# TrevorS/voxtral-mini-realtime-rs

Measured on AMD Instinct MI355X. Metric: decode_tok_per_s, higher is better.
Workload: dtype f32

## Files before the change

voxtral-mini-realtime-rs_amd/csrc/vox_engine.hip:

```cpp
#include "vox_kernels.h"

#include <hip/hip_fp16.h>

#include <cstdio>
#include <cstdlib>

namespace vox {
namespace {

#include "vox_engine_common.h"

__global__ __launch_bounds__(64) void eng_pack_lm_kernel(Q4W w, unsigned char* __restrict__ stream, size_t op_off, int vocab) {
    const int q = blockIdx.x, b = blockIdx.y, lane = threadIdx.x;
    const int row = lm_rows_per_cu(vocab) * b + q;
    unsigned char* dst = stream + (size_t)NCU * (op_off + (size_t)(q / NCONS) * PK_A) + (size_t)b * PK_A + (size_t)(q % NCONS) * PASS_A;
    const size_t src = (size_t)row * w.nb + lane;
    reinterpret_cast<uint4*>(dst)[lane] = w.qs[src];
    reinterpret_cast<uint16_t*>(dst + PA_S0)[lane] = w.sc[src];
    const size_t sh = (size_t)row * w.nb + 64 + (lane >> 1);
    const uint4 qh = w.qs[sh];
    reinterpret_cast<uint2*>(dst + PA_Q1)[lane] = (lane & 1) ? make_uint2(qh.z, qh.w) : make_uint2(qh.x, qh.y);
    if ((lane & 1) == 0) reinterpret_cast<uint16_t*>(dst + PA_S1)[lane >> 1] = w.sc[sh];
}
__global__ __launch_bounds__(64) void eng_pack_kernel(Q4W w, int op, unsigned char* __restrict__ stream, size_t op_off) {
// ... 125 lines not shown
    const EngLayerTab* tab = reinterpret_cast<const EngLayerTab*>(lds + L_TAB);
    const unsigned tag_base = (*p.serial + 1u) * 64u;
    const bool PROBE_SMALL = (p.flags & 4) != 0;
    const int own_r = min(lane0, OWN - 1);
    const unsigned own_k = (unsigned)(OWN * b + own_r);
    const float* gwt = reinterpret_cast<const float*>(lds + L_GW);
    {
        const float g0 = ld_gf(make_srd(p.n_layers > 0 ? tab[0].attn_norm : p.final_norm, ED * 4u), own_k) * (p.n_layers > 0 ? 1.0f : 512.0f);
        const float hraw = (p.flags & ENGF_ARGMAX_IN) ? comm_next_input(p, lane0, own_k) : ld_gf(make_srd(p.h_in, ED * 4u), own_k);
        comm_publish_rows(p, lane0, hraw, g0, p.H0, p.SS0, tag_base, c->h_own);
    }
#pragma unroll 1
    for (int st = 0; st <= 2 * p.n_layers; st++) {
        int lane = lane0; asm volatile("" : "+v"(lane));
        const int l = st >> 1; const bool odd = st & 1, last = st == 2 * p.n_layers, T = l == p.tl_layer;
        const unsigned tag = tag_base + (unsigned)l + 1u;
        if (odd) comm_probe_x(p, c, lane, p.H1, tag, tl, T);
        else comm_probe_x(p, c, lane, p.H0, tag - 1u, tl, false);
        lds_st(&c->gathering, 1u);
        lds_st(&c->ag_flag, (unsigned)st + 1u);
        if (T) tl(odd ? 11 : 8);
        if (p.flags & (1 | 64)) wait_ge(&c->ag_done, NCONS * ((unsigned)st + 1u), c, p.err, ERR_STAGE);
        lds_st(&c->gathering, 0u);
        if (last) break;
        if (!odd) {
            wait_ge(&c->gw_flag, (unsigned)NCONS, c, p.err, ERR_STAGE);
            const bool xloc_nt = (p.flags & 128) != 0 && (p.flags & 4096) != 0 && lds_ld(&c->xcd_ok) != 0;
            {
                wait_ge(&c->pub_cnt, NCONS * (4u * (unsigned)l + 1u), c, p.err, ERR_STAGE);
                lds_st(&c->gathering, 1u);
                float v[6];
                sweep<6>(p.G, (EQD + 2 * EKD) * 8u, tag, [&](int u) { const int i = lane + 64 * u, seg = i >> 7, e = i & 127; return seg == 0 ? 128 * h + e : (seg == 1 ? EQD : EQD + EKD) + 128 * g + e; },
                         [&]() { return lane < 32 ? EQD + 128 * g + 4 * lane : EQD + EKD + 128 * g + 4 * (lane - 32); }, PROBE_SMALL, v, c, p.err, xloc_nt);
                lds_st(&c->gathering, 0u);
#pragma unroll
                for (int u = 0; u < 6; u++) qkvn[lane + 64 * u] = v[u];
                ENG_CFENCE(); lds_st(&c->qkv_flag, (unsigned)l + 1u);
            }
            if (T) tl(9);
            {
                wait_ge(&c->pub_cnt, NCONS * (4u * (unsigned)l + 2u), c, p.err, ERR_STAGE);
                lds_st(&c->gathering, 1u);
                float v[6];
                sweep<6>(p.PW, NPW * ED * 8u, tag, [&](int u) { const int i = lane + 64 * u, hh = i / OWN, r = i - hh * OWN; return hh * ED + OWN * b + r; }, [&]() { return (lane & 31) * ED + OWN * b; }, PROBE_SMALL, v, c, p.err);
#pragma unroll
                for (int u = 0; u < 6; u++) tmp[lane + 64 * u] = v[u];
                lds_st(&c->gathering, 0u);
                ENG_CFENCE();
                float a = 0.f;
                const int r = min(lane, OWN - 1);
#pragma unroll 4
                for (int hh = 0; hh < NPW; hh++) a += tmp[hh * OWN + r];
                wait_ge(&c->gw_flag, (unsigned)NCONS, c, p.err, ERR_STAGE);
                if (!((p.flags & 16384) && blockIdx.x == 7 && l == 1))
                    comm_publish_rows(p, lane, c->h_own[r] + a, gwt[(l * 2 + 1) * 16 + r], p.H1, p.SS1, tag, c->h1_own);
            }
            if (T) tl(10);
        } else {
            const bool xloc_nt = (p.flags & 128) != 0 && (p.flags & 4096) != 0 && lds_ld(&c->xcd_ok) != 0;
            {
                wait_ge(&c->pub_cnt, NCONS * (4u * (unsigned)l + 3u), c, p.err, ERR_STAGE);
                lds_st(&c->gathering, 1u);
                float v[18];
                sweep<18>(p.A, EF * 8u, tag, [&](int u) { return 1152 * g + lane + 64 * u; }, [&]() { return 1152 * g + 36 * (lane & 31) + 35; }, PROBE_SMALL, v, c, p.err, xloc_nt);
#pragma unroll
                for (int u = 0; u < 18; u++) xa[lane + 64 * u] = v[u];
                ENG_CFENCE(); lds_st(&c->xa_flag, (unsigned)l + 1u);
                lds_st(&c->gathering, 0u);
            }
            if (T) tl(12);
            {
                wait_ge(&c->pub_cnt, NCONS * (4u * (unsigned)l + 4u), c, p.err, ERR_STAGE);
                lds_st(&c->gathering, 1u);
                float v[2];
                sweep<2>(p.P2, NP2 * ED * 8u, tag, [&](int u) { const int i = min(lane + 64 * u, NP2 * OWN - 1), pp = i / OWN, r = i - pp * OWN; return pp * ED + OWN * b + r; }, [&]() { return min(lane, NP2 - 1) * ED + OWN * b; }, PROBE_SMALL, v, c, p.err);
#pragma unroll
                for (int u = 0; u < 2; u++) if (lane + 64 * u < NP2 * OWN) tmp[lane + 64 * u] = v[u];
                lds_st(&c->gathering, 0u);
                ENG_CFENCE();
                float a = 0.f;
                const int r = min(lane, OWN - 1);
#pragma unroll
                for (int pp = 0; pp < NP2; pp++) a += tmp[pp * OWN + r];
                comm_publish_rows(p, lane, c->h1_own[r] + a, gwt[((l + 1) * 2) * 16 + r], p.H0, p.SS0, tag, c->h_own);
            }
            if (T) tl(13);
        }
    }
}

__device__ __forceinline__ f2 cvt2(unsigned w, bool hi) { return hi ? __builtin_amdgcn_cvt_pk_f32_fp8((int)w, true) : __builtin_amdgcn_cvt_pk_f32_fp8((int)w, false); }
__device__ __forceinline__ float block_dot(const uint4 q, const f2* __restrict__ x, float init) {
    f2 a0 = {init, 0.f}, a1 = {0.f, 0.f};
    const unsigned w[4] = {q.x, q.y, q.z, q.w};
#pragma unroll
    for (int d = 0; d < 4; d++) {
        const unsigned lo = w[d] & 0x0F0F0F0Fu, hi = (w[d] >> 4) & 0x0F0F0F0Fu;
        a0 = __builtin_elementwise_fma(cvt2(lo, false), x[2 * d], a0);
        a1 = __builtin_elementwise_fma(cvt2(lo, true), x[2 * d + 1], a1);
        a0 = __builtin_elementwise_fma(cvt2(hi, false), x[8 + 2 * d], a0);
        a1 = __builtin_elementwise_fma(cvt2(hi, true), x[8 + 2 * d + 1], a1);
    }
    return (a0.x + a0.y) + (a1.x + a1.y);
}

__device__ __forceinline__ float half_dot(const uint2 q, const f2* __restrict__ x, float init) {
    f2 a0 = {init, 0.f}, a1 = {0.f, 0.f};
    const unsigned w[2] = {q.x, q.y};
#pragma unroll
    for (int d = 0; d < 2; d++) {
        const unsigned lo = w[d] & 0x0F0F0F0Fu, hi = (w[d] >> 4) & 0x0F0F0F0Fu;
        a0 = __builtin_elementwise_fma(cvt2(lo, false), x[4 * d], a0);
        a1 = __builtin_elementwise_fma(cvt2(lo, true), x[4 * d + 1], a1);
        a0 = __builtin_elementwise_fma(cvt2(hi, false), x[4 * d + 2], a0);
        a1 = __builtin_elementwise_fma(cvt2(hi, true), x[4 * d + 3], a1);
    }
    return (a0.x + a0.y) + (a1.x + a1.y);
}

struct XA {
    f2 x[16], xh[8]; float m8, m8h;
    __device__ __forceinline__ void load_chunk(const float* xs, int chunk) {
        asm volatile("" : "+v"(chunk));
        const float4* x4 = reinterpret_cast<const float4*>(xs);
        float s = 0.f;
#pragma unroll
        for (int jj = 0; jj < 8; jj++) {
            const float4 v = x4[sw_piece(chunk, jj)];
            x[2 * jj] = f2{v.x, v.y}; x[2 * jj + 1] = f2{v.z, v.w};
            s += (v.x + v.y) + (v.z + v.w);
        }
        m8 = s * (-1.0f / 64.0f);
    }
    __device__ __forceinline__ void load(const float* xs, int chunk, int chunk_h, int hb) {
        load_chunk(xs, chunk);
        asm volatile("" : "+v"(chunk_h));
        const float4* x4 = reinterpret_cast<const float4*>(xs);
        float s = 0.f;
#pragma unroll
        for (int d = 0; d < 2; d++)
#pragma unroll
            for (int hh = 0; hh < 2; hh++) {
                const float4 v = x4[sw_piece(chunk_h, 4 * hh + 2 * hb + d)];
                xh[4 * d + 2 * hh] = f2{v.x, v.y}; xh[4 * d + 2 * hh + 1] = f2{v.z, v.w};
                s += (v.x + v.y) + (v.z + v.w);
            }
        m8h = s * (-1.0f / 64.0f);
    }
};
struct PassA { uint4 q0; uint2 q1; float s0, s1; };

typedef int i4v __attribute__((ext_vector_type(4)));
struct StepCtx { i4v A; float m8sx, sxinv; };
__device__ __forceinline__ StepCtx load_ctx(const unsigned char* planes, const float2* binfo, int blk0, int lane) {
    const int n = lane & 15, g = lane >> 4;
    StepCtx cx; cx.A = i4v{0, 0, 0, 0};
    if (n < 8 && (g >> 1) == (n >> 2)) cx.A = *reinterpret_cast<const i4v*>(planes + (((blk0 + (n >> 2)) * 4 + (n & 3)) * 2 + (g & 1)) * 16);
    const float2 bi = binfo[blk0 + (g & 1)];
    cx.m8sx = bi.x; cx.sxinv = bi.y;
    return cx;
}
struct RecR { i4v B; float sc; };
__device__ __forceinline__ RecR rec_read(const unsigned char* rec, bool half, int lane) {
    const int n = lane & 15, g = lane >> 4;
    uint2 q = make_uint2(0u, 0u);
    if (!half) q = reinterpret_cast<const uint2*>(rec)[lane];
    else if (n < 8) q = reinterpret_cast<const uint2*>(rec)[g * 8 + n];
    const unsigned short sb = reinterpret_cast<const unsigned short*>(rec + (half ? REC_H_SC : REC_SC))[(half ? 8 : 16) * (g & 1) + (half ? (n & 7) : n)];
    RecR r;
    r.B[0] = (int)(q.x & 0x0F0F0F0Fu); r.B[1] = (int)(q.y & 0x0F0F0F0Fu); r.B[2] = (int)((q.x >> 4) & 0x0F0F0F0Fu); r.B[3] = (int)((q.y >> 4) & 0x0F0F0F0Fu);
    r.sc = __half2float(__ushort_as_half(sb));
    asm volatile("" : "+v"(r.B[0]), "+v"(r.B[1]), "+v"(r.B[2]), "+v"(r.B[3]), "+v"(r.sc));
    return r;
}
__device__ __forceinline__ float mstep(const RecR& r, const StepCtx& cx, float acc) {
    const i4v D = __builtin_amdgcn_mfma_i32_16x16x64_i8(cx.A, r.B, i4v{0, 0, 0, 0}, 0, 0, 0);
    const int lo = (int)((unsigned)D[0] + ((unsigned)D[1] << 7)), hi = (int)((unsigned)D[2] + ((unsigned)D[3] << 7));
    float t = fmaf((float)hi, 16384.0f, (float)lo);
    t += cx.m8sx;
    return fmaf(t, r.sc * cx.sxinv, acc);
}
__device__ __forceinline__ float mstep(const unsigned char* rec, bool half, int lane, const StepCtx& cx, float acc) { return mstep(rec_read(rec, half, lane), cx, acc); }
__device__ __forceinline__ float g01_sum(float v, int lane) { return v + __shfl(v, (lane + 16) & 63); }
__device__ __forceinline__ void to_digits(const float (&v)[4], int lane, unsigned char* plane_blk, float2* binfo_blk) {
    float mx = fmaxf(fmaxf(fabsf(v[0]), fabsf(v[1])), fmaxf(fabsf(v[2]), fabsf(v[3])));
    mx = fmaxf(mx, dppf<0xB1>(mx)); mx = fmaxf(mx, dppf<0x4E>(mx)); mx = fmaxf(mx, dppf<0x141>(mx));
    int e = __builtin_amdgcn_frexp_expf(mx);
    e = max(e, -100);
    const float f = ldexpf(1.0f, 26 - e);
    int xi[4];
#pragma unroll
    for (int i = 0; i < 4; i++) xi[i] = (int)rintf(v[i] * f);
    int s = (xi[0] + xi[1]) + (xi[2] + xi[3]);
    s += dppi<0xB1>(s); s += dppi<0x4E>(s); s += dppi<0x141>(s);
    if ((lane & 7) == 0) *binfo_blk = make_float2(-8.0f * (float)s, ldexpf(1.0f, e - 26));
    const int e0 = 4 * (lane & 7), h = (e0 >> 3) & 1, off = (e0 & 4) + 8 * (e0 >> 4);
#pragma unroll
    for (int cdig = 0; cdig < 4; cdig++) {
        unsigned d = 0;
#pragma unroll
        for (int i = 0; i < 4; i++) { const int dv = cdig < 3 ? (xi[i] >> (7 * cdig)) & 127 : xi[i] >> 21; d |= (unsigned)(dv & 0xFF) << (8 * i); }
        *reinterpret_cast<unsigned*>(plane_blk + (cdig * 2 + h) * 16 + off) = d;
    }
}

struct Cons {
    const EngParams& p; EngCtl* c; unsigned char* lds; int cw, lane; unsigned P; unsigned cbar_n;
    __device__ __forceinline__ Cons(const EngParams& p_, EngCtl* c_, unsigned char* lds_, int cw_, int lane_) : p(p_), c(c_), lds(lds_), cw(cw_), lane(lane_), P(0), cbar_n(0) {}
    __device__ __forceinline__ void cbarrier() {
        cbar_n += NCONS;
        ENG_CFENCE();
        if (lane == 0) __hip_atomic_fetch_add(&c->cbar, 1u, RLX, WG);
        wait_ge(&c->cbar, cbar_n, c, p.err, ERR_CBAR);
    }
    __device__ __forceinline__ void published(const Tl& tl, int evt) {
        ENG_CFENCE();
        if (lane == 0) { const unsigned old = __hip_atomic_fetch_add(&c->pub_cnt, 1u, RLX, WG); if (evt >= 0 && tl.buf && old % NCONS == NCONS - 1) tl.buf[evt] = wall_clock64(); }
    }
    __device__ __forceinline__ const unsigned char* slot_wait(unsigned pk, int share_bytes, int& slot) {
        slot = (int)(pk % NSLOT); const unsigned k = pk / NSLOT;
        wait_ge(&c->ring_ready[slot], k + 1u, c, p.err, ERR_RING);
        return lds + L_RING + slot * SLOT_BYTES + cw * share_bytes;
    }
    __device__ __forceinline__ void slot_release(int slot) {
        ENG_CFENCE();
        if (lane == 0) __hip_atomic_fetch_add(&c->ring_done[slot], 1u, RLX, WG);
    }
    __device__ __forceinline__ void fetch(unsigned pk, PassA& P_) {
        int slot; const unsigned char* base = slot_wait(pk, PASS_A, slot);
        P_.q0 = reinterpret_cast<const uint4*>(base)[lane];
        P_.q1 = reinterpret_cast<const uint2*>(base + PA_Q1)[lane];
        P_.s0 = __half2float(__ushort_as_half(reinterpret_cast<const unsigned short*>(base + PA_S0)[lane]));
        P_.s1 = __half2float(__ushort_as_half(reinterpret_cast<const unsigned short*>(base + PA_S1)[lane >> 1]));
        slot_release(slot);
    }
    static __device__ __forceinline__ float dot(const PassA& P_, const XA& xr) { return fmaf(P_.s1, half_dot(P_.q1, xr.xh, xr.m8h), P_.s0 * block_dot(P_.q0, xr.x, xr.m8)); }

    template <bool DIGITS>
    __device__ __forceinline__ float all_gather(const u64* src, const u64* ssq, unsigned tag, unsigned stage, unsigned char* xs, float* ssl, float2* binfo, const Tl& tl, bool T) {
        wait_ge(&c->ag_flag, stage + 1u, c, p.err, ERR_STAGE);
        const srd_t sd = make_srd(src, ED * 8u), qd = make_srd(ssq, NCU * 8u);
        int ln = lane; asm volatile("" : "+v"(ln));
        if (DIGITS) {
            const unsigned q = 64u * (unsigned)cw + (unsigned)ln;
            u32x4 ra, rb; u64 rq = 0, t0 = 0;
            for (;;) {
                ra = __builtin_bit_cast(u32x4, __builtin_amdgcn_raw_buffer_load_b128(sd, (int)(q * 32u), 0, 16));
                rb = __builtin_bit_cast(u32x4, __builtin_amdgcn_raw_buffer_load_b128(sd, (int)(q * 32u + 16u), 0, 16));
                if (cw < 4) rq = ld_gran(qd, 64u * (unsigned)cw + (unsigned)ln);
                bool ok = ra.y == tag && ra.w == tag && rb.y == tag && rb.w == tag;
                if (cw < 4) ok &= (unsigned)(rq >> 32) == tag;
                if (__all(ok)) break;
                if (sweep_bail(t0, tag, c, p.err)) break;
            }
            if (T) tl(22);
            if (ln == 0) __hip_atomic_fetch_add(&c->ag_done, 1u, RLX, WG);
            const float v[4] = {__uint_as_float(ra.x), __uint_as_float(ra.z), __uint_as_float(rb.x), __uint_as_float(rb.z)};
            to_digits(v, ln, xs + (q >> 3) * 128u, binfo + (q >> 3));
            if (cw < 4) ssl[64 * cw + ln] = __uint_as_float((unsigned)rq);
            return 0.f;
        }
        const unsigned q = 64u * (((unsigned)cw + blockIdx.x) % NCONS) + (unsigned)ln;
        u32x4 ra, rb; u64 rq = 0, t0 = 0;
        for (;;) {
            ra = __builtin_bit_cast(u32x4, __builtin_amdgcn_raw_buffer_load_b128(sd, (int)(q * 32u), 0, 16));
            rb = __builtin_bit_cast(u32x4, __builtin_amdgcn_raw_buffer_load_b128(sd, (int)(q * 32u + 16u), 0, 16));
            if (cw < 4) rq = ld_gran(qd, 64u * (unsigned)cw + (unsigned)ln);
            bool ok = ra.y == tag && ra.w == tag && rb.y == tag && rb.w == tag;
            if (cw < 4) ok &= (unsigned)(rq >> 32) == tag;
            if (__all(ok)) break;
            if (sweep_bail(t0, tag, c, p.err)) break;
        }
        if (ln == 0) __hip_atomic_fetch_add(&c->ag_done, 1u, RLX, WG);
        const float v[4] = {__uint_as_float(ra.x), __uint_as_float(ra.z), __uint_as_float(rb.x), __uint_as_float(rb.z)};
#pragma unroll
        for (int i = 0; i < 4; i++) reinterpret_cast<float*>(xs)[sw_dword((int)(4u * q) + i)] = v[i];
        if (cw < 4) ssl[64 * cw + ln] = __uint_as_float((unsigned)rq);
        cbarrier();
        return rstd_staged(ssl);
    }
    __device__ __forceinline__ float rstd_staged(const float* ssl) {
        const float ss = wave_sum_e((ssl[lane] + ssl[lane + 64]) + (ssl[lane + 128] + ssl[lane + 192]));
        return 1.0f / sqrtf(ss / (float)ED + p.eps);
    }
};

__device__ __forceinline__ void eng_consumer(const EngParams& p, EngCtl* c, unsigned char* lds, int cw, const int lane0, const Tl& tl) {
    Cons cs(p, c, lds, cw, lane0);
    const int b = blockIdx.x, g = b & 7, j = b >> 3, h = 4 * g + (j >> 3), s = j & 7;
    unsigned char* xs = lds + L_XS; float* ssl = reinterpret_cast<float*>(lds + L_SSQ);
    float2* binfo = reinterpret_cast<float2*>(lds + L_BLK);
    const float* xa = reinterpret_cast<const float*>(lds + L_XA);
    float* part = reinterpret_cast<float*>(lds + L_PART);
    float* part2 = reinterpret_cast<float*>(lds + L_XA + 1152 * 4);
    const float* qkvn = reinterpret_cast<const float*>(lds + L_QKVN);
    float* sc = reinterpret_cast<float*>(lds + L_SC); float2* po = reinterpret_cast<float2*>(lds + L_PO); float* pl = reinterpret_cast<float*>(lds + L_PL);
    const unsigned tag_base = (*p.serial + 1u) * 64u;
    const int pos = *p.pos_ptr + p.pos_off + ((p.flags & ENGF_ARGMAX_IN) ? 1 : 0);
    const int j_lo = p.window >= 0 ? max(0, pos - p.window) : 0, n_old = pos - j_lo, last_old = max(n_old - 1, 0);
    const int half = EHD / 2;
    if (cw == 0 && lane0 < 24) {
        float rc = 1.0f, rs = 0.0f;
        if (lane0 < 20) { const int pr = lane0 < 16 ? 8 * s + (lane0 >> 1) : 2 * j + ((lane0 - 16) >> 1); rc = p.rope_cos[(size_t)pos * half + pr]; rs = p.rope_sin[(size_t)pos * half + pr]; }
        c->rope_c[lane0] = rc; c->rope_s[lane0] = rs;
    }
    const float scale = 1.0f / sqrtf((float)EHD);
    const int n_items = 3 * p.n_layers, npass_lm = lm_passes(p.vocab), row0_lm = lm_rows_per_cu(p.vocab) * b;
    {
        const EngLayerTab* tab = reinterpret_cast<const EngLayerTab*>(lds + L_TAB);
        float* gwt = reinterpret_cast<float*>(lds + L_GW);
        const bool xchg = cw == NCONS - 1 && (p.flags & 128) != 0;
        const unsigned my = c->xcc_id;
        if (xchg && lane0 == 0) publish(p.XC + b, tag_base, __uint_as_float(my));
        const int l = cw + NCONS * (lane0 >> 4), r = lane0 & 15, lc = min(l, max(p.n_layers - 1, 0));
        const bool lok = r < OWN && l <= p.n_layers && (lane0 >> 4) < 3, lay = l < p.n_layers;
        const unsigned k = (unsigned)(OWN * b + min(r, OWN - 1));
        const gcf_p pa = as_g(lay ? tab[lc].attn_norm : p.final_norm);
        float wa = 0.f, wf = 0.f, wd = 0.f;
        if (lok) { wa = pa[k]; if (p.n_layers > 0) { wf = as_g(tab[lc].ffn_norm)[k]; wd = as_g(tab[lc].ada_mul)[k]; } }
        if (lok) {
            gwt[(l * 2) * 16 + r] = lay ? wa : wa * 512.0f;
            if (lay) gwt[(l * 2 + 1) * 16 + r] = wf * wd;
        }
        if (cw == NCONS - 1) {
            unsigned ok = 0;
            if (xchg) {
                float v[1];
                const bool got = sweep<1>(p.XC, NCU * 8u, tag_base, [&](int) { return 8 * (lane0 & 31) + g; }, [&]() { return 0; }, false, v, c, p.err);
                ok = got && __all(__float_as_uint(v[0]) == my) ? 1u : 0u;
                if (!ok && lane0 == 0) __hip_atomic_store(p.err + 1, 9u | ((unsigned)b << 8) | (my << 16), RLX, AG);
            }
            lds_st(&c->xcd_ok, ok);
        }
        ENG_CFENCE();
        if (lane0 == 0) __hip_atomic_fetch_add(&c->gw_flag, 1u, RLX, WG);
    }
    float best = -INFINITY; int best_i = 0x7fffffff;
    bool xloc = false;

#pragma unroll 1
    for (int it = 0; it <= n_items; it++) {
        int lane = lane0; asm volatile("" : "+v"(lane));
        const int l = it / 3, op = it == n_items ? (int)EOP_LM : (it - 3 * l == 0 ? (int)EOP_QKV : it - 3 * l == 1 ? (int)EOP_W13 : (int)EOP_W2);
        const bool T = l == p.tl_layer && cw == 0 && op != EOP_LM;
        const int tlev = l == p.tl_layer ? 1 : 0;
        const unsigned tag = tag_base + (unsigned)l + 1u;
        const EngLayerTab* L = reinterpret_cast<const EngLayerTab*>(lds + L_TAB) + (op == EOP_LM ? 0 : l);
        if (op == EOP_QKV) {
            const gf_p kc = as_g(L->kc) + (size_t)g * p.max_seq * EHD, vc = as_g(L->vc) + (size_t)g * p.max_seq * EHD;
            const int t12 = cw * 64 + lane;
            const int part_ = t12 & 7, ks = t12 >> 3;
            RecR rq[8];
            {
                int s0, s1, s2;
                const unsigned char* b0 = cs.slot_wait(cs.P, 2 * REC, s0);
                rq[0] = rec_read(b0, false, lane); rq[1] = rec_read(b0 + REC, false, lane);
                cs.slot_release(s0);
                const unsigned char* b1 = cs.slot_wait(cs.P + 1, 2 * REC, s1);
                rq[2] = rec_read(b1, false, lane); rq[3] = rec_read(b1 + REC, false, lane);
                cs.slot_release(s1);
                const unsigned char* b2 = cs.slot_wait(cs.P + 2, 4 * REC_H, s2);
#pragma unroll
                for (int i = 0; i < 4; i++) rq[4 + i] = rec_read(b2 + i * REC_H, true, lane);
                cs.slot_release(s2);
                cs.P += QKV_PK;
            }
            cs.all_gather<true>(p.H0, p.SS0, tag - 1u, 2u * (unsigned)l, xs, ssl, binfo, tl, false);
            if (T) tl(0);
            constexpr int NKP = 2;
            float4 kpre[NKP][4];
            auto kload = [&](int u) {
                const unsigned ko = (unsigned)(j_lo + min(ks + 96 * u, last_old)) * EHD + part_ * 16;
#pragma unroll
                for (int e = 0; e < 4; e++) kpre[u][e] = make_float4(0.f, 0.f, 0.f, 0.f);
                if (ks + 96 * u < n_old) {
#pragma unroll
                    for (int e = 0; e < 4; e++) kpre[u][e] = ldg4(kc + (ko + 4 * e));
                }
            };
            kload(0);
            {
                float a0 = 0.f, a1 = 0.f;
#pragma unroll
                for (int i = 0; i < 4; i++) {
                    const StepCtx cx = load_ctx(xs, binfo, 2 * (4 * cw + i), lane);
                    a0 = mstep(rq[i], cx, a0); a1 = mstep(rq[4 + i], cx, a1);
                }
                a0 = g01_sum(a0, lane); a1 = g01_sum(a1, lane);
                if (lane < 16) part[lane * NCONS + cw] = a0;
                if (lane < 8) part[(16 + lane) * NCONS + cw] = a1;
            }
            cs.cbarrier();
            if (it == 0) { wait_ge(&c->gw_flag, (unsigned)NCONS, c, p.err, ERR_STAGE); xloc = (p.flags & 128) != 0 && lds_ld(&c->xcd_ok) != 0; }
            if (cw == 0) {
                const int r = min(lane, 23);
                float a = 0.f;
#pragma unroll
                for (int w = 0; w < NCONS; w++) a += part[r * NCONS + w];
                a *= cs.rstd_staged(ssl);
                const float rc = c->rope_c[r], rs = c->rope_s[r];
                const float o = dppf<0xB1>(a);
                const float y = (lane & 1) ? fmaf(o, rs, a * rc) : fmaf(-o, rs, a * rc);
                if (lane < 24) {
                    const int n = lane < 16 ? 128 * h + 16 * s + lane : lane < 20 ? EQD + 128 * g + 4 * j + (lane - 16) : EQD + EKD + 128 * g + 4 * j + (lane - 20);
                    publish_b(p.G, (EQD + 2 * EKD) * 8u, (unsigned)n, tag, y, xloc);
                    if (lane >= 16) (lane < 20 ? kc : vc)[(size_t)pos * EHD + (n & 127)] = y;
                }
            }
            cs.published(tl, tlev ? 28 : -1);
            if (T) tl(1);
            kload(1);
            float2 vpre[16];
#pragma unroll
            for (int u = 0; u < 16; u++) {
                vpre[u] = make_float2(0.f, 0.f);
                if (cw + 12 * u < n_old) {
                    const fv2 v = *(const __attribute__((address_space(1))) fv2*)(vc + ((unsigned)(j_lo + cw + 12 * u) * EHD + lane * 2));
                    vpre[u] = make_float2(v.x, v.y);
                }
            }
            wait_ge(&c->qkv_flag, (unsigned)l + 1u, c, p.err, ERR_STAGE);
            if (T) tl(2);
            {
                float qv[16];
#pragma unroll
                for (int e = 0; e < 4; e++) { const float4 v = *reinterpret_cast<const float4*>(qkvn + part_ * 16 + 4 * e); qv[4 * e] = v.x; qv[4 * e + 1] = v.y; qv[4 * e + 2] = v.z; qv[4 * e + 3] = v.w; }
                auto dot16 = [&](const float4 (&kk)[4]) {
                    float sacc = 0.f;
#pragma unroll
                    for (int e = 0; e < 4; e++) { sacc = fmaf(qv[4 * e], kk[e].x, sacc); sacc = fmaf(qv[4 * e + 1], kk[e].y, sacc); sacc = fmaf(qv[4 * e + 2], kk[e].z, sacc); sacc = fmaf(qv[4 * e + 3], kk[e].w, sacc); }
                    return group8_sum_e(sacc);
                };
#pragma unroll
                for (int u = 0; u < NKP; u++) {
                    const float sv = dot16(kpre[u]);
                    const int i = ks + 96 * u;
                    if (part_ == 0 && i < n_old) sc[i] = sv * scale;
                }
                for (int i0 = 96 * NKP; i0 < n_old; i0 += 96 * NKP) {
#pragma unroll
                    for (int u = 0; u < NKP; u++) {
                        const int i = i0 + ks + 96 * u;
                        const unsigned ko = (unsigned)(j_lo + min(i, last_old)) * EHD + part_ * 16;
#pragma unroll
                        for (int e = 0; e < 4; e++) kpre[u][e] = make_float4(0.f, 0.f, 0.f, 0.f);
                        if (i < n_old) {
#pragma unroll
                            for (int e = 0; e < 4; e++) kpre[u][e] = ldg4(kc + (ko + 4 * e));
                        }
                    }
#pragma unroll
                    for (int u = 0; u < NKP; u++) {
                        const float sv = dot16(kpre[u]);
                        const int i = i0 + ks + 96 * u;
                        if (part_ == 0 && i < n_old) sc[i] = sv * scale;
                    }
                }
                if (cw == 0) {
                    float4 kk[4];
#pragma unroll
                    for (int e = 0; e < 4; e++) kk[e] = *reinterpret_cast<const float4*>(qkvn + 128 + part_ * 16 + 4 * e);
                    const float sv = dot16(kk);
                    if (t12 == 0) sc[n_old] = sv * scale;
                }
            }
            if (T) tl(26);
            cs.cbarrier();
            if (T) tl(27);
            {
                const int n = n_old + 1;
                float mx = -INFINITY;
                for (int i = lane; i < n; i += 64) mx = fmaxf(mx, sc[i]);
                mx = wave_max_e(mx);
                float2 o = make_float2(0.f, 0.f); float lsum = 0.f;
                const int iu = cw + 12 * (lane & 15);
                const float pv = iu < n_old ? expf(sc[iu] - mx) : 0.f;
#pragma unroll
                for (int u = 0; u < 16; u++) {
                    const float pr_ = rlf(pv, u); const float2 vv = vpre[u];
                    o.x = fmaf(pr_, vv.x, o.x); o.y = fmaf(pr_, vv.y, o.y); lsum += pr_;
                }
                for (int b0 = 192; b0 < n_old; b0 += 192) {
#pragma unroll
                    for (int u = 0; u < 16; u++) {
                        vpre[u] = make_float2(0.f, 0.f);
                        if (b0 + cw + 12 * u < n_old) {
                            const fv2 v = *(const __attribute__((address_space(1))) fv2*)(vc + ((unsigned)(j_lo + b0 + cw + 12 * u) * EHD + lane * 2));
                            vpre[u] = make_float2(v.x, v.y);
                        }
                    }
                    const int ib = b0 + cw + 12 * (lane & 15);
                    const float pb = ib < n_old ? expf(sc[ib] - mx) : 0.f;
#pragma unroll
                    for (int u = 0; u < 16; u++) {
                        const float pr_ = rlf(pb, u); const float2 vv = vpre[u];
                        o.x = fmaf(pr_, vv.x, o.x); o.y = fmaf(pr_, vv.y, o.y); lsum += pr_;
                    }
                }
                if (cw == 0) {
                    const float pr_ = expf(sc[n_old] - mx); const float2 vv = *reinterpret_cast<const float2*>(qkvn + 256 + lane * 2);
                    o.x = fmaf(pr_, vv.x, o.x); o.y = fmaf(pr_, vv.y, o.y); lsum += pr_;
                }
                po[cw * 64 + lane] = o;
                if (lane == 0) pl[cw] = lsum;
            }
            if (T) tl(23);
            cs.cbarrier();
            if (T) tl(25);
            if (lane < 32) {
                const float4* po4 = reinterpret_cast<const float4*>(po);
                float4 so = make_float4(0.f, 0.f, 0.f, 0.f); float sl = 0.f;
#pragma unroll
                for (int q = 0; q < 12; q++) { const float4 a = po4[q * 32 + lane]; so.x += a.x; so.y += a.y; so.z += a.z; so.w += a.w; sl += pl[q]; }
                const float inv = 1.0f / sl;
                const float v[4] = {so.x * inv, so.y * inv, so.z * inv, so.w * inv};
                to_digits(v, lane, xs + (8 * cw + (lane >> 3)) * 128, binfo + 8 * cw + (lane >> 3));
            }
            if (T) tl(3);
            {
                StepCtx cx[2];
#pragma unroll
                for (int i = 0; i < 2; i++) cx[i] = load_ctx(xs, binfo, 8 * cw + 2 * i, lane);
#pragma unroll
                for (int i = 0; i < WO_PK; i++) {
                    int sl_; const unsigned char* bb = cs.slot_wait(cs.P + i, 2 * REC, sl_);
                    float a = mstep(bb, false, lane, cx[0], 0.f); a = mstep(bb + REC, false, lane, cx[1], a);
                    cs.slot_release(sl_);
                    a = g01_sum(a, lane);
                    if (lane < 16) publish_b(p.PW, NPW * ED * 8u, (unsigned)(h * ED + 384 * s + 16 * (2 * cw + i) + lane), tag, a, false);
                }
                cs.P += WO_PK;
                cs.published(tl, tlev ? 29 : -1);
            }
            if (T) tl(4);
            continue;
        }
        if (op == EOP_W13) {
            constexpr int NPRE = 3;
            RecR rw[4 * NPRE];
#pragma unroll
            for (int ti = 0; ti < NPRE; ti++) {
                int s0, s1;
                const unsigned char* b0 = cs.slot_wait(cs.P + 2 * ti, 2 * REC, s0);
                rw[4 * ti] = rec_read(b0, false, lane); rw[4 * ti + 1] = rec_read(b0 + REC, false, lane);
                cs.slot_release(s0);
                const unsigned char* b1 = cs.slot_wait(cs.P + 2 * ti + 1, 2 * REC, s1);
                rw[4 * ti + 2] = rec_read(b1, false, lane); rw[4 * ti + 3] = rec_read(b1 + REC, false, lane);
                cs.slot_release(s1);
            }
            cs.all_gather<true>(p.H1, p.SS1, tag, 2u * (unsigned)l + 1u, xs, ssl, binfo, tl, T);
            if (T) tl(5);
            StepCtx cx[4];
#pragma unroll
            for (int i = 0; i < 4; i++) cx[i] = load_ctx(xs, binfo, 2 * (4 * cw + i), lane);
            if (T) tl(24);
#pragma unroll
            for (int ti = 0; ti < NPRE; ti++) {
                float a = 0.f;
#pragma unroll
                for (int i = 0; i < 4; i++) a = mstep(rw[4 * ti + i], cx[i], a);
                a = g01_sum(a, lane);
                if (lane < 16) part[(16 * ti + lane) * NCONS + cw] = a;
            }
#pragma unroll 1
            for (int ti = NPRE; ti < 4; ti++) {
                int s0, s1;
                const unsigned char* b0 = cs.slot_wait(cs.P + 2 * ti, 2 * REC, s0);
                const unsigned char* b1 = cs.slot_wait(cs.P + 2 * ti + 1, 2 * REC, s1);
                float a = mstep(b0, false, lane, cx[0], 0.f); a = mstep(b0 + REC, false, lane, cx[1], a);
                a = mstep(b1, false, lane, cx[2], a); a = mstep(b1 + REC, false, lane, cx[3], a);
                cs.slot_release(s0); cs.slot_release(s1);
                a = g01_sum(a, lane);
                if (lane < 16) part[(16 * ti + lane) * NCONS + cw] = a;
            }
            {
                int s2; const unsigned char* b2 = cs.slot_wait(cs.P + 8, 4 * REC_H, s2);
                float a = 0.f;
#pragma unroll
                for (int i = 0; i < 4; i++) a = mstep(b2 + i * REC_H, true, lane, cx[i], a);
                cs.slot_release(s2);
                a = g01_sum(a, lane);
                if (lane < 8) part[(64 + lane) * NCONS + cw] = a;
            }
            cs.P += W13_PK;
            cs.cbarrier();
            if (cw < 2) {
                const int r = min(64 * cw + lane, 71);
                float a = 0.f;
#pragma unroll
                for (int w = 0; w < NCONS; w++) a += part[r * NCONS + w];
                a *= cs.rstd_staged(ssl);
                const float up = dppf<0xB1>(a);
                if ((lane & 1) == 0 && 64 * cw + lane < 72) publish_b(p.A, EF * 8u, (unsigned)(1152 * g + 36 * j + (r >> 1)), tag, silu_e(a) * up, xloc);
            }
            cs.published(tl, tlev ? 30 : -1);
            if (T) tl(6);
            continue;
        }
        if (op == EOP_W2) {
            RecR r2[9];
#pragma unroll
            for (int i = 0; i < W2_PK; i++) {
                int sl_; const unsigned char* bb = cs.slot_wait(cs.P + i, 3 * REC, sl_);
#pragma unroll
                for (int k = 0; k < 3; k++) r2[3 * i + k] = rec_read(bb + k * REC, false, lane);
                cs.slot_release(sl_);
            }
            wait_ge(&c->xa_flag, (unsigned)l + 1u, c, p.err, ERR_STAGE);
            if (T) tl(7);
            const int ksl = cw % 6, tg = cw / 6;
            if (lane < 48) {
                const float4 v4 = *reinterpret_cast<const float4*>(xa + 32 * (6 * ksl + (lane >> 3)) + 4 * (lane & 7));
                const float v[4] = {v4.x, v4.y, v4.z, v4.w};
                to_digits(v, lane, xs + (8 * cw + (lane >> 3)) * 128, binfo + 8 * cw + (lane >> 3));
            }
            StepCtx cx[3];
#pragma unroll
            for (int i = 0; i < 3; i++) cx[i] = load_ctx(xs, binfo, 8 * cw + 2 * i, lane);
#pragma unroll
            for (int i = 0; i < W2_PK; i++) {
                float a = mstep(r2[3 * i], cx[0], 0.f); a = mstep(r2[3 * i + 1], cx[1], a); a = mstep(r2[3 * i + 2], cx[2], a);
                a = g01_sum(a, lane);
                if (lane < 16) part2[(16 * (3 * tg + i) + lane) * 6 + ksl] = a;
            }
            cs.P += W2_PK;
            cs.cbarrier();
            if (cw < 2) {
                const int r = min(64 * cw + lane, 95);
                float a = 0.f;
#pragma unroll
                for (int w = 0; w < 6; w++) a += part2[r * 6 + w];
                if (64 * cw + lane < 96) publish_b(p.P2, NP2 * ED * 8u, (unsigned)(g * ED + 96 * j + r), tag, a, false);
            }
            cs.published(tl, tlev ? 31 : -1);
            if (T) tl(14);
            continue;
        }
        const float rstd = cs.all_gather<false>(p.H0, p.SS0, tag_base + (unsigned)p.n_layers, 2u * (unsigned)p.n_layers, xs, ssl, binfo, tl, false);
        XA xr; xr.load(reinterpret_cast<const float*>(xs), lane, 64 + (lane >> 1), lane & 1);
        const int n_pass = lm_packets(p.vocab);
        PassA Qa, Qb;
        cs.fetch(cs.P, Qa);
#pragma unroll 1
        for (int t = 0; t < n_pass; t++) {
            const int q = cw + NCONS * t;
            if (t + 1 < n_pass) cs.fetch(cs.P + t + 1, Qb);
            if (q < npass_lm) {
                const float r = wave_sum_e(Cons::dot(Qa, xr)) * rstd;
                const int n = row0_lm + q;
                if (p.logits_out && lane == 0) p.logits_out[n] = r;
                if (r > best || (r == best && n < best_i)) { best = r; best_i = n; }
            }
            Qa = Qb;
        }
        cs.P += (unsigned)n_pass;
    }
    if (lane0 == 0) { c->best_val[cw] = best; c->best_idx[cw] = best_i; }
    cs.cbarrier();
    if (cw == 0 && lane0 == 0) {
        float bv = c->best_val[0]; int bi = c->best_idx[0];
        for (int w = 1; w < NCONS; w++) { const float v = c->best_val[w]; const int ii = c->best_idx[w]; if (v > bv || (v == bv && ii < bi)) { bv = v; bi = ii; } }
        p.part_val[b] = bv; p.part_idx[b] = bi;
    }
    if (cw == 0) tl(15);
}

__global__ __launch_bounds__(NTHR, 1) void decode_engine_kernel(const EngParams p) {
    extern __shared__ __attribute__((aligned(16))) unsigned char lds[];
    EngCtl* c = reinterpret_cast<EngCtl*>(lds + L_CTL);
    const int tid = threadIdx.x, lane = tid & 63, wave = __builtin_amdgcn_readfirstlane(tid >> 6);
    if (tid < (int)(sizeof(EngCtl) / 4)) reinterpret_cast<unsigned*>(c)[tid] = 0u;
    for (int i = tid; i < p.n_layers * (int)(sizeof(EngLayerTab) / 8); i += NTHR) reinterpret_cast<u64*>(lds + L_TAB)[i] = reinterpret_cast<const u64*>(p.layers)[i];
    if (tid == 0) c->xcc_id = __builtin_amdgcn_s_getreg((20) | (0 << 6) | ((4 - 1) << 11));
    __syncthreads();
    Tl tl; tl.on = p.tl != nullptr && lane == 0; tl.buf = p.tl ? p.tl + (size_t)blockIdx.x * 32 : nullptr;
    if (wave == 0) {
        tl(19);
        eng_loader(p, c, (unsigned)(uintptr_t)(lds + L_RING), lane, tl);
    } else if (wave == 1) {
        eng_comm(p, c, lds, lane, tl);
        if (blockIdx.x == 0 && lane == 0) {
            const unsigned sv = *p.serial; asm volatile("" ::: "memory"); *p.serial = sv + 1u;
            if (p.flags & ENGF_ARGMAX_IN) { const int pv_ = *p.pos_rw; asm volatile("" ::: "memory"); *p.pos_rw = pv_ + 1; }
        }
    } else {
        eng_consumer(p, c, lds, wave - 2, lane, tl);
    }
}

__global__ __launch_bounds__(256) void eng_hidden_kernel(const u64* __restrict__ H, const u64* __restrict__ SS, float eps, float* __restrict__ out) {
    __shared__ float red[256];
    const int t = threadIdx.x;
    red[t] = __uint_as_float((unsigned)SS[t]);
    __syncthreads();
    for (int s = 128; s > 0; s >>= 1) { if (t < s) red[t] += red[t + s]; __syncthreads(); }
    const float rstd = 1.0f / sqrtf(red[0] / (float)ED + eps);
    const int k = blockIdx.x * 256 + t;
    out[k] = __uint_as_float((unsigned)H[k]) * (1.0f / 512.0f) * rstd;
}

}

hipError_t launch_eng_hidden(const EngParams& p, float* out, hipStream_t s) {
    const bool even = ((2 * p.n_layers) & 1) == 0;
    eng_hidden_kernel<<<dim3(ED / 256), dim3(256), 0, s>>>(even ? p.H0 : p.H1, even ? p.SS0 : p.SS1, p.eps, out);
    return hipGetLastError();
}

bool eng_geometry_ok(int D, int n_heads, int n_kv, int hd, int ffn, int vocab, int max_seq) {
    return D == ED && n_heads == ENH && n_kv == ENKV && hd == EHD && ffn == EF && vocab > 0 && vocab % NCU == 0 && max_seq > 0 && max_seq <= SC_MAX;
}
size_t eng_stream_bytes(int n_layers, int vocab) { return cu_stream_bytes(n_layers, vocab) * NCU; }
int eng_lds_bytes() { return L_TOTAL; }

static constexpr size_t ST_H0 = 0, ST_H1 = ST_H0 + (size_t)ED * 8, ST_G = ST_H1 + (size_t)ED * 8, ST_PW = ST_G + (size_t)(EQD + 2 * EKD) * 8,
                        ST_A = ST_PW + (size_t)NPW * ED * 8, ST_P2 = ST_A + (size_t)EF * 8, ST_SS0 = ST_P2 + (size_t)NP2 * ED * 8, ST_SS1 = ST_SS0 + (size_t)NCU * 8, ST_XC = ST_SS1 + (size_t)NCU * 8, ST_SERIAL = ST_XC + (size_t)NCU * 8, ST_ERR = ST_SERIAL + 256, ST_TOTAL = ST_ERR + 256;
size_t eng_state_bytes() { return ST_TOTAL; }
void eng_state_carve(unsigned char* st, EngParams* p) {
    p->H0 = reinterpret_cast<unsigned long long*>(st + ST_H0); p->H1 = reinterpret_cast<unsigned long long*>(st + ST_H1);
    p->XC = reinterpret_cast<unsigned long long*>(st + ST_XC);
    p->SS0 = reinterpret_cast<unsigned long long*>(st + ST_SS0); p->SS1 = reinterpret_cast<unsigned long long*>(st + ST_SS1);
    p->G = reinterpret_cast<unsigned long long*>(st + ST_G); p->PW = reinterpret_cast<unsigned long long*>(st + ST_PW);
    p->A = reinterpret_cast<unsigned long long*>(st + ST_A); p->P2 = reinterpret_cast<unsigned long long*>(st + ST_P2);
    p->serial = reinterpret_cast<unsigned*>(st + ST_SERIAL); p->err = reinterpret_cast<unsigned*>(st + ST_ERR);
}

hipError_t launch_eng_pack(const Q4W& w, int op, int layer, int n_layers, unsigned char* stream, int vocab, hipStream_t s) {
    if (w.fmt != WFMT_Q4_0 || !w.qs || !w.sc) return hipErrorInvalidValue;
    int off_bytes, N, K;
    switch (op) {
    case EOP_QKV: off_bytes = OFF_QKV; N = EQD + 2 * EKD; K = ED; break;
    case EOP_WO: off_bytes = OFF_WO; N = ED; K = EQD; break;
    case EOP_W13: off_bytes = OFF_W13; N = 2 * EF; K = ED; break;
    case EOP_W2: off_bytes = OFF_W2; N = ED; K = EF; break;
    case EOP_LM: off_bytes = 0; N = vocab; K = ED; break;
    case EOP_WOB: off_bytes = 0; N = ED; K = EQD; break;
    default: return hipErrorInvalidValue;
    }
    if (w.N != N || w.K != K) return hipErrorInvalidValue;
    if (op == EOP_LM) eng_pack_lm_kernel<<<dim3(lm_passes(vocab), NCU), dim3(64), 0, s>>>(w, stream, (size_t)n_layers * LAYER_BYTES, vocab);
    else if (op == EOP_WOB) eng_pack_kernel<<<dim3(op_packets(op) * NCONS * 4, NCU), dim3(64), 0, s>>>(w, op, stream, (size_t)layer * WOB_LAYER_BYTES);
    else eng_pack_kernel<<<dim3(op_packets(op) * NCONS * 4, NCU), dim3(64), 0, s>>>(w, op, stream, (size_t)layer * LAYER_BYTES + off_bytes);
    return hipGetLastError();
}

hipError_t eng_occupancy(int* blocks_per_cu) {
    hipError_t e = hipFuncSetAttribute(reinterpret_cast<const void*>(decode_engine_kernel), hipFuncAttributeMaxDynamicSharedMemorySize, 160 * 1024);
    if (e != hipSuccess) return e;
    return hipOccupancyMaxActiveBlocksPerMultiprocessor(blocks_per_cu, reinterpret_cast<const void*>(decode_engine_kernel), NTHR, L_TOTAL);
}

hipError_t launch_decode_engine(const EngParams& p, hipStream_t s) {
    static DevOnce attr_done;
    const int dev = vox_current_device();
    if (!attr_done.done(dev)) {
        hipError_t e = hipFuncSetAttribute(reinterpret_cast<const void*>(decode_engine_kernel), hipFuncAttributeMaxDynamicSharedMemorySize, 160 * 1024);
        if (e != hipSuccess) return e;
        attr_done.set(dev);
    }
    decode_engine_kernel<<<dim3(NCU), dim3(NTHR), L_TOTAL, s>>>(p);
    attn_form_note(ATTN_FORM_ENGINE);
    return hipGetLastError();
}

}
```

Measured before the change: 1513.

## Pair K-steps into chained MFMA calls with permlane-swap reductions

Restructures the int8 MFMA GEMV steps so that two K-blocks are processed per accumulation, using two chained 16x16x64 MFMAs (lo/hi A halves) feeding one digit-recombination and scale FMA. Cross-group reduction switches from a shuffle to permlane32/permlane16 swaps summing four groups. The aim is to halve the post-MFMA scalar recombination work and the shuffle reductions in QKV, WO, W13 and W2. W2 gets a custom pairing with a leftover half-step. The cost is more register pressure from the paired records and more complex lane masking.

```diff
diff --git a/voxtral-mini-realtime-rs_amd/csrc/vox_engine.hip b/voxtral-mini-realtime-rs_amd/csrc/vox_engine.hip
--- a/voxtral-mini-realtime-rs_amd/csrc/vox_engine.hip
+++ b/voxtral-mini-realtime-rs_amd/csrc/vox_engine.hip
@@ -301,14 +301,6 @@
 
 typedef int i4v __attribute__((ext_vector_type(4)));
 struct StepCtx { i4v A; float m8sx, sxinv; };
-__device__ __forceinline__ StepCtx load_ctx(const unsigned char* planes, const float2* binfo, int blk0, int lane) {
-    const int n = lane & 15, g = lane >> 4;
-    StepCtx cx; cx.A = i4v{0, 0, 0, 0};
-    if (n < 8 && (g >> 1) == (n >> 2)) cx.A = *reinterpret_cast<const i4v*>(planes + (((blk0 + (n >> 2)) * 4 + (n & 3)) * 2 + (g & 1)) * 16);
-    const float2 bi = binfo[blk0 + (g & 1)];
-    cx.m8sx = bi.x; cx.sxinv = bi.y;
-    return cx;
-}
 struct RecR { i4v B; float sc; };
 __device__ __forceinline__ RecR rec_read(const unsigned char* rec, bool half, int lane) {
     const int n = lane & 15, g = lane >> 4;
@@ -329,8 +321,53 @@
     t += cx.m8sx;
     return fmaf(t, r.sc * cx.sxinv, acc);
 }
-__device__ __forceinline__ float mstep(const unsigned char* rec, bool half, int lane, const StepCtx& cx, float acc) { return mstep(rec_read(rec, half, lane), cx, acc); }
-__device__ __forceinline__ float g01_sum(float v, int lane) { return v + __shfl(v, (lane + 16) & 63); }
+struct PairCtx { i4v Alo, Ahi; float m8sx, sxinv; };
+__device__ __forceinline__ PairCtx load_ctx2(const unsigned char* planes, const float2* binfo, int blk_a, int blk_b, int lane) {
+    const int n = lane & 15, g = lane >> 4, p = (n & 7) >> 2;
+    i4v X = i4v{0, 0, 0, 0};
+    if ((g >> 1) == p) X = *reinterpret_cast<const i4v*>(planes + ((((n < 8 ? blk_a : blk_b) + p) * 4 + (n & 3)) * 2 + (g & 1)) * 16);
+    PairCtx cx;
+#pragma unroll
+    for (int i = 0; i < 4; i++) { cx.Alo[i] = n < 8 ? X[i] : 0; cx.Ahi[i] = n < 8 ? 0 : X[i]; }
+    const float2 bi = binfo[(g < 2 ? blk_a : blk_b) + (g & 1)];
+    cx.m8sx = bi.x; cx.sxinv = bi.y;
+    return cx;
+}
+struct RecP { i4v Ba, Bb; float sc; };
+__device__ __forceinline__ RecP rec_read2(const unsigned char* rec_a, const unsigned char* rec_b, bool half, int lane) {
+    const int n = lane & 15, g = lane >> 4;
+    uint2 qa = make_uint2(0u, 0u), qb = make_uint2(0u, 0u);
+    if (!half) { qa = reinterpret_cast<const uint2*>(rec_a)[lane]; qb = reinterpret_cast<const uint2*>(rec_b)[lane]; }
+    else if (n < 8) { qa = reinterpret_cast<const uint2*>(rec_a)[g * 8 + n]; qb = reinterpret_cast<const uint2*>(rec_b)[g * 8 + n]; }
+    const unsigned short sb = reinterpret_cast<const unsigned short*>((g < 2 ? rec_a : rec_b) + (half ? REC_H_SC : REC_SC))[(half ? 8 : 16) * (g & 1) + (half ? (n & 7) : n)];
+    RecP r;
+    r.Ba[0] = (int)(qa.x & 0x0F0F0F0Fu); r.Ba[1] = (int)(qa.y & 0x0F0F0F0Fu); r.Ba[2] = (int)((qa.x >> 4) & 0x0F0F0F0Fu); r.Ba[3] = (int)((qa.y >> 4) & 0x0F0F0F0Fu);
+    r.Bb[0] = (int)(qb.x & 0x0F0F0F0Fu); r.Bb[1] = (int)(qb.y & 0x0F0F0F0Fu); r.Bb[2] = (int)((qb.x >> 4) & 0x0F0F0F0Fu); r.Bb[3] = (int)((qb.y >> 4) & 0x0F0F0F0Fu);
+    r.sc = __half2float(__ushort_as_half(sb));
+    asm volatile("" : "+v"(r.Ba[0]), "+v"(r.Ba[1]), "+v"(r.Ba[2]), "+v"(r.Ba[3]), "+v"(r.Bb[0]), "+v"(r.Bb[1]), "+v"(r.Bb[2]), "+v"(r.Bb[3]), "+v"(r.sc));
+    return r;
+}
+__device__ __forceinline__ RecR rec_read_lo(const unsigned char* rec, int lane) {
+    RecR r = rec_read(rec, false, lane);
+    r.sc = lane < 32 ? r.sc : 0.f;
+    asm volatile("" : "+v"(r.sc));
+    return r;
+}
+__device__ __forceinline__ float mstep2(const RecP& r, const PairCtx& cx, float acc) {
+    i4v D = __builtin_amdgcn_mfma_i32_16x16x64_i8(cx.Alo, r.Ba, i4v{0, 0, 0, 0}, 0, 0, 0);
+    D = __builtin_amdgcn_mfma_i32_16x16x64_i8(cx.Ahi, r.Bb, D, 0, 0, 0);
+    const int lo = (int)((unsigned)D[0] + ((unsigned)D[1] << 7)), hi = (int)((unsigned)D[2] + ((unsigned)D[3] << 7));
+    float t = fmaf((float)hi, 16384.0f, (float)lo);
+    t += cx.m8sx;
+    return fmaf(t, r.sc * cx.sxinv, acc);
+}
+__device__ __forceinline__ float mstep2(const unsigned char* rec_a, const unsigned char* rec_b, bool half, int lane, const PairCtx& cx, float acc) { return mstep2(rec_read2(rec_a, rec_b, half, lane), cx, acc); }
+__device__ __forceinline__ float g4_sum(float v) {
+    const auto a = __builtin_amdgcn_permlane32_swap(__float_as_uint(v), __float_as_uint(v), false, false);
+    const float w = __uint_as_float(a[0]) + __uint_as_float(a[1]);
+    const auto b = __builtin_amdgcn_permlane16_swap(__float_as_uint(w), __float_as_uint(w), false, false);
+    return __uint_as_float(b[0]) + __uint_as_float(b[1]);
+}
 __device__ __forceinline__ void to_digits(const float (&v)[4], int lane, unsigned char* plane_blk, float2* binfo_blk) {
     float mx = fmaxf(fmaxf(fabsf(v[0]), fabsf(v[1])), fmaxf(fabsf(v[2]), fabsf(v[3])));
     mx = fmaxf(mx, dppf<0xB1>(mx)); mx = fmaxf(mx, dppf<0x4E>(mx)); mx = fmaxf(mx, dppf<0x141>(mx));
@@ -499,18 +536,18 @@
             const gf_p kc = as_g(L->kc) + (size_t)g * p.max_seq * EHD, vc = as_g(L->vc) + (size_t)g * p.max_seq * EHD;
             const int t12 = cw * 64 + lane;
             const int part_ = t12 & 7, ks = t12 >> 3;
-            RecR rq[8];
+            RecP rq[4];
             {
                 int s0, s1, s2;
                 const unsigned char* b0 = cs.slot_wait(cs.P, 2 * REC, s0);
-                rq[0] = rec_read(b0, false, lane); rq[1] = rec_read(b0 + REC, false, lane);
+                rq[0] = rec_read2(b0, b0 + REC, false, lane);
                 cs.slot_release(s0);
                 const unsigned char* b1 = cs.slot_wait(cs.P + 1, 2 * REC, s1);
-                rq[2] = rec_read(b1, false, lane); rq[3] = rec_read(b1 + REC, false, lane);
+                rq[1] = rec_read2(b1, b1 + REC, false, lane);
                 cs.slot_release(s1);
                 const unsigned char* b2 = cs.slot_wait(cs.P + 2, 4 * REC_H, s2);
 #pragma unroll
-                for (int i = 0; i < 4; i++) rq[4 + i] = rec_read(b2 + i * REC_H, true, lane);
+                for (int i = 0; i < 2; i++) rq[2 + i] = rec_read2(b2 + 2 * i * REC_H, b2 + (2 * i + 1) * REC_H, true, lane);
                 cs.slot_release(s2);
                 cs.P += QKV_PK;
             }
@@ -531,11 +568,11 @@
             {
                 float a0 = 0.f, a1 = 0.f;
 #pragma unroll
-                for (int i = 0; i < 4; i++) {
-                    const StepCtx cx = load_ctx(xs, binfo, 2 * (4 * cw + i), lane);
-                    a0 = mstep(rq[i], cx, a0); a1 = mstep(rq[4 + i], cx, a1);
-                }
-                a0 = g01_sum(a0, lane); a1 = g01_sum(a1, lane);
+                for (int i = 0; i < 2; i++) {
+                    const PairCtx cx = load_ctx2(xs, binfo, 8 * cw + 4 * i, 8 * cw + 4 * i + 2, lane);
+                    a0 = mstep2(rq[i], cx, a0); a1 = mstep2(rq[2 + i], cx, a1);
+                }
+                a0 = g4_sum(a0); a1 = g4_sum(a1);
                 if (lane < 16) part[lane * NCONS + cw] = a0;
                 if (lane < 8) part[(16 + lane) * NCONS + cw] = a1;
             }
@@ -667,15 +704,13 @@
             }
             if (T) tl(3);
             {
-                StepCtx cx[2];
-#pragma unroll
-                for (int i = 0; i < 2; i++) cx[i] = load_ctx(xs, binfo, 8 * cw + 2 * i, lane);
+                const PairCtx cx = load_ctx2(xs, binfo, 8 * cw, 8 * cw + 2, lane);
 #pragma unroll
                 for (int i = 0; i < WO_PK; i++) {
                     int sl_; const unsigned char* bb = cs.slot_wait(cs.P + i, 2 * REC, sl_);
-                    float a = mstep(bb, false, lane, cx[0], 0.f); a = mstep(bb + REC, false, lane, cx[1], a);
+                    float a = mstep2(bb, bb + REC, false, lane, cx, 0.f);
                     cs.slot_release(sl_);
-                    a = g01_sum(a, lane);
+                    a = g4_sum(a);
                     if (lane < 16) publish_b(p.PW, NPW * ED * 8u, (unsigned)(h * ED + 384 * s + 16 * (2 * cw + i) + lane), tag, a, false);
                 }
                 cs.P += WO_PK;
@@ -686,29 +721,27 @@
         }
         if (op == EOP_W13) {
             constexpr int NPRE = 3;
-            RecR rw[4 * NPRE];
+            RecP rw[2 * NPRE];
 #pragma unroll
             for (int ti = 0; ti < NPRE; ti++) {
                 int s0, s1;
                 const unsigned char* b0 = cs.slot_wait(cs.P + 2 * ti, 2 * REC, s0);
-                rw[4 * ti] = rec_read(b0, false, lane); rw[4 * ti + 1] = rec_read(b0 + REC, false, lane);
+                rw[2 * ti] = rec_read2(b0, b0 + REC, false, lane);
                 cs.slot_release(s0);
                 const unsigned char* b1 = cs.slot_wait(cs.P + 2 * ti + 1, 2 * REC, s1);
-                rw[4 * ti + 2] = rec_read(b1, false, lane); rw[4 * ti + 3] = rec_read(b1 + REC, false, lane);
+                rw[2 * ti + 1] = rec_read2(b1, b1 + REC, false, lane);
                 cs.slot_release(s1);
             }
             cs.all_gather<true>(p.H1, p.SS1, tag, 2u * (unsigned)l + 1u, xs, ssl, binfo, tl, T);
             if (T) tl(5);
-            StepCtx cx[4];
-#pragma unroll
-            for (int i = 0; i < 4; i++) cx[i] = load_ctx(xs, binfo, 2 * (4 * cw + i), lane);
+            PairCtx cx[2];
+#pragma unroll
+            for (int i = 0; i < 2; i++) cx[i] = load_ctx2(xs, binfo, 8 * cw + 4 * i, 8 * cw + 4 * i + 2, lane);
             if (T) tl(24);
 #pragma unroll
             for (int ti = 0; ti < NPRE; ti++) {
-                float a = 0.f;
-#pragma unroll
-                for (int i = 0; i < 4; i++) a = mstep(rw[4 * ti + i], cx[i], a);
-                a = g01_sum(a, lane);
+                float a = mstep2(rw[2 * ti], cx[0], 0.f); a = mstep2(rw[2 * ti + 1], cx[1], a);
+                a = g4_sum(a);
                 if (lane < 16) part[(16 * ti + lane) * NCONS + cw] = a;
             }
 #pragma unroll 1
@@ -716,19 +749,16 @@
                 int s0, s1;
                 const unsigned char* b0 = cs.slot_wait(cs.P + 2 * ti, 2 * REC, s0);
                 const unsigned char* b1 = cs.slot_wait(cs.P + 2 * ti + 1, 2 * REC, s1);
-                float a = mstep(b0, false, lane, cx[0], 0.f); a = mstep(b0 + REC, false, lane, cx[1], a);
-                a = mstep(b1, false, lane, cx[2], a); a = mstep(b1 + REC, false, lane, cx[3], a);
+                float a = mstep2(b0, b0 + REC, false, lane, cx[0], 0.f); a = mstep2(b1, b1 + REC, false, lane, cx[1], a);
                 cs.slot_release(s0); cs.slot_release(s1);
-                a = g01_sum(a, lane);
+                a = g4_sum(a);
                 if (lane < 16) part[(16 * ti + lane) * NCONS + cw] = a;
             }
             {
                 int s2; const unsigned char* b2 = cs.slot_wait(cs.P + 8, 4 * REC_H, s2);
-                float a = 0.f;
-#pragma unroll
-                for (int i = 0; i < 4; i++) a = mstep(b2 + i * REC_H, true, lane, cx[i], a);
+                float a = mstep2(b2, b2 + REC_H, true, lane, cx[0], 0.f); a = mstep2(b2 + 2 * REC_H, b2 + 3 * REC_H, true, lane, cx[1], a);
                 cs.slot_release(s2);
-                a = g01_sum(a, lane);
+                a = g4_sum(a);
                 if (lane < 8) part[(64 + lane) * NCONS + cw] = a;
             }
             cs.P += W13_PK;
@@ -747,13 +777,20 @@
             continue;
         }
         if (op == EOP_W2) {
-            RecR r2[9];
-#pragma unroll
-            for (int i = 0; i < W2_PK; i++) {
-                int sl_; const unsigned char* bb = cs.slot_wait(cs.P + i, 3 * REC, sl_);
-#pragma unroll
-                for (int k = 0; k < 3; k++) r2[3 * i + k] = rec_read(bb + k * REC, false, lane);
-                cs.slot_release(sl_);
+            static_assert(W2_PK == 3, "w2's pairing is written out for three tiles of three K-steps per wave");
+            RecP r2[3], r2s; RecR r2l;
+            {
+                int s0, s1, s2;
+                const unsigned char* b0 = cs.slot_wait(cs.P, 3 * REC, s0);
+                r2[0] = rec_read2(b0, b0 + REC, false, lane);
+                const unsigned char* b1 = cs.slot_wait(cs.P + 1, 3 * REC, s1);
+                r2[1] = rec_read2(b1, b1 + REC, false, lane);
+                r2s = rec_read2(b0 + 2 * REC, b1 + 2 * REC, false, lane);
+                cs.slot_release(s0); cs.slot_release(s1);
+                const unsigned char* b2 = cs.slot_wait(cs.P + 2, 3 * REC, s2);
+                r2[2] = rec_read2(b2, b2 + REC, false, lane);
+                r2l = rec_read_lo(b2 + 2 * REC, lane);
+                cs.slot_release(s2);
             }
             wait_ge(&c->xa_flag, (unsigned)l + 1u, c, p.err, ERR_STAGE);
             if (T) tl(7);
@@ -763,14 +800,19 @@
                 const float v[4] = {v4.x, v4.y, v4.z, v4.w};
                 to_digits(v, lane, xs + (8 * cw + (lane >> 3)) * 128, binfo + 8 * cw + (lane >> 3));
             }
-            StepCtx cx[3];
-#pragma unroll
-            for (int i = 0; i < 3; i++) cx[i] = load_ctx(xs, binfo, 8 * cw + 2 * i, lane);
-#pragma unroll
-            for (int i = 0; i < W2_PK; i++) {
-                float a = mstep(r2[3 * i], cx[0], 0.f); a = mstep(r2[3 * i + 1], cx[1], a); a = mstep(r2[3 * i + 2], cx[2], a);
-                a = g01_sum(a, lane);
-                if (lane < 16) part2[(16 * (3 * tg + i) + lane) * 6 + ksl] = a;
+            const PairCtx cxp = load_ctx2(xs, binfo, 8 * cw, 8 * cw + 2, lane), cxs = load_ctx2(xs, binfo, 8 * cw + 4, 8 * cw + 4, lane);
+            {
+                const float m = mstep2(r2s, cxs, 0.f);
+                float a[3];
+                a[0] = mstep2(r2[0], cxp, lane < 32 ? m : 0.f);
+                a[1] = mstep2(r2[1], cxp, lane < 32 ? 0.f : m);
+                a[2] = mstep2(r2[2], cxp, 0.f);
+                a[2] = mstep(r2l, StepCtx{cxs.Alo, cxs.m8sx, cxs.sxinv}, a[2]);
+#pragma unroll
+                for (int i = 0; i < W2_PK; i++) {
+                    const float t = g4_sum(a[i]);
+                    if (lane < 16) part2[(16 * (3 * tg + i) + lane) * 6 + ksl] = t;
+                }
             }
             cs.P += W2_PK;
             cs.cbarrier();
```

New measurement: 1531, median of 6. 1.2% higher.
